# aleju/face-generator

Measured on NVIDIA H100. Metric: 32x32 GAN train images/sec (1 D-iter + 1 G-iter per batch, batch 256/GPU), higher is better.
Workload: dtype f32

## Files before the change

### face_generator_b200/csrc/capi.cu

```cuda
#include <algorithm>
#include <cstdarg>
#include <cstdlib>
#include <cstring>

#include "fg_internal.h"
#include "k_conv_tc.h"

static thread_local char g_err[1024] = "";
void fg_set_error(const char* fmt, ...) {
  va_list ap;
  va_start(ap, fmt);
  vsnprintf(g_err, sizeof(g_err), fmt, ap);
  va_end(ap);
}

#define ENTER(c)                                      \
  do {                                                \
    if (!(c)) {                                       \
      fg_set_error("null fg_ctx");                    \
      return FG_ERR_INVALID;                          \
    }                                                 \
    FG_CUDA(cudaSetDevice((c)->device));              \
  } while (0)

// ... 232 lines not shown
  ENTER(c);
  c->graph_epoch++;
  if (!strcmp(key, "sgd_momentum_D") || !strcmp(key, "sgd_momentum_G")) {
    FG_REQUIRE(v >= 0.0 && v < 1.0, "%s must be in [0, 1)", key);
    (key[13] == 'D' ? c->sgd_mom_D : c->sgd_mom_G) = (float)v;
    return FG_OK;
  }
  fg_set_error("fg_set_option_f: unknown key '%s'", key);
  return FG_ERR_INVALID;
}
int64_t fg_get_option(fg_ctx* c, const char* key) {
  if (!c || !key) return -1;
  if (!strcmp(key, "conv_impl")) return c->conv_impl;
  if (!strcmp(key, "max_batch")) return c->maxB;
  if (!strcmp(key, "channels")) return c->C;
  if (!strcmp(key, "sm_count")) return c->sm_count;
  if (!strcmp(key, "bn_epilogue")) return c->bn_epilogue;
  if (!strcmp(key, "edge_impl")) return c->edge_impl;
  if (!strcmp(key, "mma_f16")) return c->mma_f16;
  if (!strcmp(key, "dp_overlap")) return c->dp_overlap;
  if (!strcmp(key, "use_graph")) return c->use_graph;
  if (!strcmp(key, "bwd_merge")) return c->bwd_merge;
  if (!strcmp(key, "bwd_merge_ctas")) return c->bwd_merge_ctas;
  if (!strcmp(key, "optimizer_D")) return c->opt_D;
  if (!strcmp(key, "optimizer_G")) return c->opt_G;
  if (!strcmp(key, "last_conv_kind")) return c->last_conv_kind;
  if (!strcmp(key, "last_conv_tile_m")) return c->last_conv_tile_m;
  if (!strcmp(key, "last_conv_tile_n")) return c->last_conv_tile_n;
  if (!strcmp(key, "last_conv_format")) return c->last_conv_format;
  if (!strcmp(key, "last_conv_splits")) return c->last_conv_splits;
  return -1;
}

int fg_adam_step(fg_ctx* c, float* p, const float* g, float* m, float* v, int64_t n, float lr, float beta1, float beta2,
                 float eps, int t, float l1_grad, float l2, float clampv, float grad_scale) {
  ENTER(c);
  FG_REQUIRE(p && g && m && v && n > 0 && t >= 1, "fg_adam_step: bad arguments");
  const double step = (double)lr * sqrt(1.0 - pow((double)beta2, t)) / (1.0 - pow((double)beta1, t));
  return k_adam(c, p, g, m, v, n, beta1, beta2, eps, l1_grad, l2, clampv, grad_scale, nullptr, nullptr, (float)step,
                nullptr);
}

void* fg_dev_alloc(size_t bytes) {
  void* p = nullptr;
  if (cudaMalloc(&p, bytes) != cudaSuccess) {
    fg_set_error("fg_dev_alloc(%zu) failed: %s", bytes, cudaGetErrorString(cudaGetLastError()));
// ... 93 lines not shown
```

### face_generator_b200/csrc/fg_internal.h

```cpp
#pragma once
#include <cuda_runtime.h>
#include <cstdint>
#include <cstdio>
#include <deque>
#include <functional>
#include <initializer_list>
#include <map>
#include <string>
#include <vector>

#include "fg_b200.h"

void fg_set_error(const char* fmt, ...);

#define FG_CUDA(call)                                                                               \
  do {                                                                                              \
    cudaError_t e__ = (call);                                                                       \
    if (e__ != cudaSuccess) {                                                                       \
      fg_set_error("%s:%d: %s -> %s", __FILE__, __LINE__, #call, cudaGetErrorString(e__));          \
      return FG_ERR_CUDA;                                                                           \
    }                                                                                               \
  } while (0)
#define FG_TRY(call)                  \
  do {                                \
// ... 192 lines not shown
  double* red_ws = nullptr;
  size_t red_ws_elems = 0;
  double* red_ws_opt = nullptr;
  unsigned* red_ticket = nullptr;
  double* bn_slice_acc = nullptr;
  float* bn_parts = nullptr;
  int edge_impl = 1;
  int bn_epilogue = 1;
  int mma_f16 = 1;
  float* lop_sx = nullptr;
  float* lop_sy = nullptr;
  unsigned* amax_out = nullptr;
  bool* amax_done = nullptr;
  double* bn_acc = nullptr;
  float* io_dev = nullptr;
  size_t io_dev_elems = 0;
  float* scratch[8] = {nullptr, nullptr, nullptr, nullptr, nullptr, nullptr, nullptr, nullptr};
  size_t scratch_elems[8] = {0, 0, 0, 0, 0, 0, 0, 0};
  void* nccl_comm = nullptr;
  int world = 1, rank = 0;
  int dp_overlap = 1;
  int reserve_sms = 0;
  int last_conv_kind = 0, last_conv_tile_m = 0, last_conv_tile_n = 0, last_conv_format = 0, last_conv_splits = 0;
  int bwd_merge = 1, bwd_merge_ctas = 0;
  int* bwd_claim = nullptr;
  int use_graph = 1, graph_epoch = 0;
  uint64_t* seed_dev = nullptr;
  cudaStream_t comm_stream = nullptr;
  cudaEvent_t ev_fork = nullptr, ev_join = nullptr;
  bool debug_keep = false;
  cudaEvent_t events[16] = {};
  bool timing = false;
  std::map<std::string, TimerRec> timers;
};

inline void note_conv(fg_ctx* c, int kind, int tile_m, int tile_n, int format, int splits) {
  c->last_conv_kind = kind;
  c->last_conv_tile_m = tile_m;
  c->last_conv_tile_n = tile_n;
  c->last_conv_format = format;
  c->last_conv_splits = splits;
}

struct ScopedTimer {
  fg_ctx* c;
  TimerRec* rec = nullptr;
  cudaEvent_t e0 = nullptr, e1 = nullptr;
// ... 197 lines not shown
```

### face_generator_b200/csrc/k_conv_tc.cu

```cuda
#include <cuda.h>
#include <cuda_fp16.h>

#include <algorithm>
#include <cstdlib>
#include <cstring>
#include <functional>
#include <queue>
#include <vector>

#include "fg_internal.h"
#include "k_conv_tc.h"
#include "k_f16split.cuh"
#include "k_wgmma.cuh"

namespace {

__device__ __forceinline__ uint32_t smem_u32(const void* p) { return (uint32_t)__cvta_generic_to_shared(p); }

__device__ __forceinline__ void mbar_init(uint64_t* bar, uint32_t count) {
  asm volatile("mbarrier.init.shared::cta.b64 [%0], %1;" ::"r"(smem_u32(bar)), "r"(count));
}
__device__ __forceinline__ void mbar_expect_tx(uint64_t* bar, uint32_t bytes) {
  asm volatile("mbarrier.arrive.expect_tx.shared::cta.b64 _, [%0], %1;" ::"r"(smem_u32(bar)), "r"(bytes) : "memory");
}
// ... 339 lines not shown
bool pick_box(int H, int W, int npix, int* bw, int* bh, int* bb) {
  if (W <= 0 || H <= 0) return false;
  if (W >= npix) {
    if (W % npix) return false;
    *bw = npix; *bh = 1; *bb = 1;
    return true;
  }
  if (npix % W) return false;
  const int rows = npix / W;
  if (rows <= H) {
    if (H % rows) return false;
    *bw = W; *bh = rows; *bb = 1;
    return true;
  }
  if (rows % H) return false;
  *bw = W; *bh = H; *bb = rows / H;
  return true;
}

template <int BN>
constexpr size_t fwd_smem() { return (size_t)kStages * (2 * kABytes + 2 * BN * 128) + 256 + 5 * 8 * BN * 4 + 1024; }
template <int BN>
constexpr size_t wg_smem() { return (size_t)3 * (2 * 4 * 4096 + 2 * (BN / 32) * 4096) + 128 + 1024; }
template <int BN>
constexpr size_t bwd_smem() { return (size_t)kStages * fwd_stage_bytes<BN>() + 256 + 1024; }


template <int N, bool F16 = false>
__global__ void __launch_bounds__(256, 1) tf32_peak_kernel(int iters, float* sink) {
  extern __shared__ uint8_t smem_raw[];
  uint8_t* smem = reinterpret_cast<uint8_t*>((reinterpret_cast<uintptr_t>(smem_raw) + 1023) & ~(uintptr_t)1023);
  constexpr uint32_t kFoot = (128 + N) * 128;
  for (uint32_t i = threadIdx.x; i < kFoot / 4; i += blockDim.x) reinterpret_cast<float*>(smem)[i] = 1.f;
  asm volatile("fence.proxy.async.shared::cta;" ::: "memory");
  __syncthreads();
  const uint32_t sa = smem_u32(smem);
  const uint64_t a = make_desc(sa + (threadIdx.x >> 7) * 64 * 128, 16, 1024), b = make_desc(sa + 128 * 128, 16, 1024);
  float acc[N / 2];
#pragma unroll
  for (int i = 0; i < N / 2; ++i) acc[i] = 0.f;
  for (int i = 0; i < iters; ++i) {
    wgmma_fence();
#pragma unroll
    for (int k = 0; k < 4; ++k) wgmma_op<N, F16, false>(acc, a + (uint64_t)(k * 2), b + (uint64_t)(k * 2), 1);
    wgmma_commit();
    wgmma_wait<1>();
  }
  wgmma_wait<0>();
// ... 31 lines not shown
  cudaEventDestroy(e1);
  const double flops = (double)c->sm_count * iters * 4.0 * 2.0 * 128 * N * (f16 ? 16 : 8);
  *tflops = flops / (best * 1e-3) / 1e12;
  return FG_OK;
}

int tc_encode_nhwc_box(CUtensorMap* m, const float* base, int C, int W, int H, int B, int bc, int bw, int bh, int bb) {
  FG_TRY(get_encode());
  const int64_t sW = (int64_t)C * 4, sH = sW * W, sB = sH * H;
  return make_map4(m, base, C, W, H, B, sW, sH, sB, bc, bw, bh, bb, CU_TENSOR_MAP_SWIZZLE_NONE);
}

int tc_init(fg_ctx* c) {
  (void)c;
  FG_TRY(get_encode());
  FG_CUDA(cudaFuncSetAttribute(tapconv_tc_kernel<64>, cudaFuncAttributeMaxDynamicSharedMemorySize, (int)fwd_smem<64>()));
  FG_CUDA(cudaFuncSetAttribute(tapconv_tc_kernel<128>, cudaFuncAttributeMaxDynamicSharedMemorySize, (int)fwd_smem<128>()));
  FG_CUDA(cudaFuncSetAttribute(tapconv_tc_kernel<64, true>, cudaFuncAttributeMaxDynamicSharedMemorySize, (int)fwd_smem<64>()));
  FG_CUDA(cudaFuncSetAttribute(tapconv_tc_kernel<128, true>, cudaFuncAttributeMaxDynamicSharedMemorySize, (int)fwd_smem<128>()));
  FG_CUDA(cudaFuncSetAttribute(wgrad_tc_kernel<64>, cudaFuncAttributeMaxDynamicSharedMemorySize, (int)wg_smem<64>()));
  FG_CUDA(cudaFuncSetAttribute(wgrad_tc_kernel<128>, cudaFuncAttributeMaxDynamicSharedMemorySize, (int)wg_smem<128>()));
  FG_CUDA(cudaFuncSetAttribute(wgrad_tc_kernel<64, true>, cudaFuncAttributeMaxDynamicSharedMemorySize, (int)wg_smem<64>()));
  FG_CUDA(cudaFuncSetAttribute(wgrad_tc_kernel<128, true>, cudaFuncAttributeMaxDynamicSharedMemorySize, (int)wg_smem<128>()));
  FG_CUDA(cudaFuncSetAttribute(bwd_pair_tc_kernel<128>, cudaFuncAttributeMaxDynamicSharedMemorySize, (int)bwd_smem<128>()));
  return FG_OK;
}
void tc_destroy(fg_ctx* c) { (void)c; }

int tc_split(fg_ctx* c, const float* x, float* hi, float* lo, int64_t n) {
  if (n % 4) {
    fg_set_error("tc_split: element count must be a multiple of 4");
    return FG_ERR_INVALID;
  }
  int64_t g = (n / 4 + 255) / 256;
  if (g > kGridCap) g = kGridCap;
  if (reinterpret_cast<uintptr_t>(x) % 16 == 0) split_kernel<true><<<(int)g, 256, 0, c->stream>>>(x, hi, lo, n / 4);
  else split_kernel<false><<<(int)g, 256, 0, c->stream>>>(x, hi, lo, n / 4);
  LAUNCH_CHECK(c);
  return FG_OK;
}
int tc_amax(fg_ctx* c, const float* x, int64_t n, float* amax_slot) {
  if (n % 4 || reinterpret_cast<uintptr_t>(x) % 16) {
    fg_set_error("tc_amax: needs a 16-byte aligned tensor with a multiple of 4 elements");
    return FG_ERR_INVALID;
  }
  FG_CUDA(cudaMemsetAsync(amax_slot, 0, 2 * sizeof(float), c->stream));
  int64_t g = (n / 4 + 255) / 256;
// ... 179 lines not shown
  FG_TRY(make_map2(&p.b_lo, w_lo, g.Cin, (int64_t)ntapw * g.Cout, ke, BN, false, h));
  p.kpt = g.Cin / ke;
  p.oscale = oscale ? oscale : oscale2;
  p.oscale2 = oscale ? oscale2 : nullptr;
  p.Cout = g.Cout;
  p.B = g.B; p.H = Hl; p.W = Wl;
  p.tiles_x = Wl / p.bw;
  p.tiles_y = Hl / p.bh;
  p.tiles_per_phase = p.bb == 1 ? g.B * p.tiles_x * p.tiles_y : (g.B + p.bb - 1) / p.bb;
  p.out = out;
  p.bias = bias;
  p.stats = stats;
  if (n_parts) *n_parts = p.tiles_per_phase * p.nphase;
  p.out_H = g.H; p.out_W = g.W;
  p.out_scale = g.ups;
  p.ntiles = p.tiles_per_phase * p.nphase * (g.Cout / BN);
  p.chunk = tc_chunk(g.H * g.W > 1);
  if (f16 && g.H * g.W == 1) p.chunk = std::max(1, p.chunk / 2);
  return launch_tapconv(c, p, BN, f16);
}


static int dgrad_ups_params(const float* dy_hi, const float* dy_lo, const float* wd_hi, const float* wd_lo, float* out,
                            ConvGeom g, int f16, const float* oscale, TcFwdParams& p, int* BN_out) {
  memset(&p, 0, sizeof(p));
  const int Hl = g.H / 2, Wl = g.W / 2;
  if (!pick_box(Hl, Wl, 128, &p.bw, &p.bh, &p.bb)) return FG_ERR_UNSUPPORTED;
  const int Cy = g.Cout;
  const int es = f16 ? 2 : 4, ke = f16 ? 64 : 32;
  const bool h = f16 != 0;
  if (Cy % ke) return FG_ERR_UNSUPPORTED;
  for (int ph = 0; ph < 4; ++ph) {
    const int py = ph >> 1, px = ph & 1;
    const int64_t off_bytes = ((int64_t)py * g.W + px) * Cy * es;
    const float* b_hi = reinterpret_cast<const float*>(reinterpret_cast<const char*>(dy_hi) + off_bytes);
    const float* b_lo = reinterpret_cast<const float*>(reinterpret_cast<const char*>(dy_lo) + off_bytes);
    const int64_t sW = (int64_t)2 * Cy * es, sH = (int64_t)2 * g.W * Cy * es, sB = (int64_t)g.H * g.W * Cy * es;
    FG_TRY(make_map4(&p.a_hi[ph], b_hi, Cy, Wl, Hl, g.B, sW, sH, sB, ke, p.bw, p.bh, p.bb, CU_TENSOR_MAP_SWIZZLE_128B, false, h));
    FG_TRY(make_map4(&p.a_lo[ph], b_lo, Cy, Wl, Hl, g.B, sW, sH, sB, ke, p.bw, p.bh, p.bb, CU_TENSOR_MAP_SWIZZLE_128B, false, h));
  }
  const int BN = g.Cin % 128 == 0 ? 128 : 64;
  p.nphase = 1;
  p.ntaps = 36;
  for (int ph = 0; ph < 4; ++ph)
    for (int t = 0; t < 9; ++t) {
      p.dy[ph * 9 + t] = (int8_t)(1 - t / 3);
      p.dx[ph * 9 + t] = (int8_t)(1 - t % 3);
      p.amap[ph * 9 + t] = (int8_t)ph;
      p.widx[ph * 9 + t] = (int16_t)(ph * 9 + t);
    }
  FG_TRY(make_map2(&p.b_hi, wd_hi, Cy, (int64_t)36 * g.Cin, ke, BN, false, h));
  FG_TRY(make_map2(&p.b_lo, wd_lo, Cy, (int64_t)36 * g.Cin, ke, BN, false, h));
  p.kpt = Cy / ke;
  p.oscale = oscale;
  p.Cout = g.Cin;
  p.B = g.B; p.H = Hl; p.W = Wl;
  p.tiles_x = Wl / p.bw;
  p.tiles_y = Hl / p.bh;
  p.tiles_per_phase = p.bb == 1 ? g.B * p.tiles_x * p.tiles_y : (g.B + p.bb - 1) / p.bb;
  p.out = out;
  p.bias = nullptr;
  p.out_H = Hl; p.out_W = Wl;
  p.out_scale = 1;
  p.ntiles = p.tiles_per_phase * (g.Cin / BN);
  p.chunk = tc_chunk(true);
  *BN_out = BN;
  return FG_OK;
}
int tc_conv_dgrad_ups(fg_ctx* c, const float* dy_hi, const float* dy_lo, const float* wd_hi, const float* wd_lo,
                      float* out, ConvGeom g, int f16, const float* oscale) {
  TcFwdParams p;
  int BN;
  FG_TRY(dgrad_ups_params(dy_hi, dy_lo, wd_hi, wd_lo, out, g, f16, oscale, p, &BN));
  return launch_tapconv(c, p, BN, f16);
}

static int wgrad_splits(const fg_ctx* c, int base, int kblocks) {
  const int splits = std::min(std::max(1, c->sm_count / base), kblocks);
  const int per = (kblocks + splits - 1) / splits;
  return (kblocks + per - 1) / per;
}

static int wgrad_params(fg_ctx* c, const float* x_hi, const float* x_lo, const float* dy_hi, const float* dy_lo, ConvGeom g,
                        int f16, const float* oscale, const float* oscale2, TcWgParams& p, int* BN_out, int* ntt_out,
                        int* splits_out) {
  memset(&p, 0, sizeof(p));
  const int Hl = g.H / g.ups, Wl = g.W / g.ups;
  const bool h = f16 != 0;
  const int es = h ? 2 : 4, gch = h ? 64 : 32;
  if (!pick_box(Hl, Wl, h ? 64 : 32, &p.bw, &p.bh, &p.bb)) return FG_ERR_UNSUPPORTED;
  if (g.Cin % 64 || g.Cout % 128) return FG_ERR_UNSUPPORTED;
  const int BN = g.Cin % 128 == 0 ? 128 : 64;
  {
    const int64_t sW = (int64_t)g.Cin * es, sH = sW * Wl, sB = sH * Hl;
    const int ngx = BN / gch;
    FG_TRY(make_map5(&p.x_hi, x_hi, g.Cin, Wl, Hl, g.B, sW, sH, sB, p.bw, p.bh, p.bb, ngx, h));
// ... 63 lines not shown
  if (f16) {
    if (BN == 128) wgrad_tc_kernel<128, true><<<grid, kTcThreads, wg_smem<128>(), c->stream>>>(p);
    else wgrad_tc_kernel<64, true><<<grid, kTcThreads, wg_smem<64>(), c->stream>>>(p);
  } else if (BN == 128) wgrad_tc_kernel<128><<<grid, kTcThreads, wg_smem<128>(), c->stream>>>(p);
  else wgrad_tc_kernel<64><<<grid, kTcThreads, wg_smem<64>(), c->stream>>>(p);
  LAUNCH_CHECK(c);
  return splits > 1 ? k_splitk_reduce(c, c->splitk_ws, splits, size, out) : FG_OK;
}

bool tc_bwd_pair_eligible(const fg_ctx* c, const ConvGeom& g) {
  int bw, bh, bb;
  const int Hl = g.H / 2, Wl = g.W / 2;
  if (g.ups != 2 || g.k != 5 || g.Cin % 128 || g.Cout % 128) return false;
  if (!pick_box(Hl, Wl, 128, &bw, &bh, &bb) || !pick_box(Hl, Wl, 64, &bw, &bh, &bb)) return false;
  const int kblocks = bb == 1 ? g.B * (Wl / bw) * (Hl / bh) : (g.B + bb - 1) / bb;
  return wgrad_splits(c, 36 * (g.Cout / 128) * (g.Cin / 128), kblocks) == 1;
}

static int bwd_pair_ctas(const fg_ctx* c, int nitems) {
  int ctas = std::min(nitems, std::max(1, c->sm_count - c->reserve_sms));
  return c->bwd_merge_ctas > 0 ? std::min(ctas, c->bwd_merge_ctas) : ctas;
}

bool tc_bwd_pair_pays(const fg_ctx* c, const ConvGeom& g) {
  if (!tc_bwd_pair_eligible(c, g)) return false;
  int bw, bh, bb, tw, th, tb;
  const int Hl = g.H / 2, Wl = g.W / 2;
  pick_box(Hl, Wl, 64, &bw, &bh, &bb);
  pick_box(Hl, Wl, 128, &tw, &th, &tb);
  const int64_t wlen = bb == 1 ? g.B * (Wl / bw) * (Hl / bh) : (g.B + bb - 1) / bb;
  const int64_t dlen = 36 * (g.Cout / 64);
  const int nwg = 36 * (g.Cout / 128) * (g.Cin / 128);
  const int ntiles = (tb == 1 ? g.B * (Wl / tw) * (Hl / th) : (g.B + tb - 1) / tb) * (g.Cin / 128);
  const int sms = std::max(1, c->sm_count - c->reserve_sms);
  const int64_t two = wlen + (int64_t)((ntiles + sms - 1) / sms) * dlen;
  std::priority_queue<int64_t, std::vector<int64_t>, std::greater<int64_t>> free_at;
  for (int i = 0, n = bwd_pair_ctas(c, nwg + ntiles); i < n; ++i) free_at.push(0);
  int64_t merged = 0;
  for (int id = 0; id < nwg + ntiles; ++id) {
    const int64_t end = free_at.top() + (id < nwg ? wlen : dlen);
    free_at.pop();
    free_at.push(end);
    merged = std::max(merged, end);
  }
  return merged * 20 < two * 19;
}

int tc_conv_bwd_ups(fg_ctx* c, const float* x_hi, const float* x_lo, const float* dy_hi, const float* dy_lo,
                    const float* wd_hi, const float* wd_lo, float* wg_out, float* dh, ConvGeom g, const float* oscale_dy,
                    const float* oscale_x) {
  if (!tc_bwd_pair_eligible(c, g)) {
    fg_set_error("tc_conv_bwd_ups: no merged backward for Cin %d, Cout %d at %dx%d, batch %d", g.Cin, g.Cout, g.H, g.W, g.B);
    return FG_ERR_UNSUPPORTED;
  }
  TcBwdParams p;
  memset(&p, 0, sizeof(p));
  int wBN, ntt, splits, dBN;
  FG_TRY(wgrad_params(c, x_hi, x_lo, dy_hi, dy_lo, g, 1, oscale_dy, oscale_x, p.wg, &wBN, &ntt, &splits));
  FG_TRY(dgrad_ups_params(dy_hi, dy_lo, wd_hi, wd_lo, dh, g, 1, oscale_dy, p.dg, &dBN));
  if (wBN != 128 || dBN != 128 || splits != 1) {
    fg_set_error("tc_conv_bwd_ups: unexpected tiling (wgrad BN %d, %d splits, dgrad BN %d)", wBN, splits, dBN);
    return FG_ERR_UNSUPPORTED;
  }
  p.wg.out = wg_out;
  p.wg.split_stride = 0;
  p.claim = c->bwd_claim;
  p.nwg = ntt * (g.Cout / 128) * (g.Cin / 128);
  p.nitems = p.nwg + p.dg.ntiles;
  const int ctas = bwd_pair_ctas(c, p.nitems);
  FG_CUDA(cudaMemsetAsync(c->bwd_claim, 0, sizeof(int), c->stream));
  bwd_pair_tc_kernel<128><<<ctas, kTcThreads, bwd_smem<128>(), c->stream>>>(p);
  LAUNCH_CHECK(c);
  return FG_OK;
}
```

### face_generator_b200/csrc/k_conv_tc_kernels.cuh

```cuda
#pragma once

constexpr int kConsumerThreads = 256;
constexpr int kTcThreads = kConsumerThreads + 128;

__device__ __forceinline__ void wgmma_fence() { asm volatile("wgmma.fence.sync.aligned;" ::: "memory"); }
__device__ __forceinline__ void wgmma_commit() { asm volatile("wgmma.commit_group.sync.aligned;" ::: "memory"); }
template <int N>
__device__ __forceinline__ void wgmma_wait() { asm volatile("wgmma.wait_group.sync.aligned %0;" ::"n"(N) : "memory"); }
__device__ __forceinline__ void consumer_sync() { asm volatile("bar.sync 1, %0;" ::"n"(kConsumerThreads) : "memory"); }
__device__ __forceinline__ void producer_regs() { asm volatile("setmaxnreg.dec.sync.aligned.u32 40;" ::: "memory"); }
__device__ __forceinline__ void consumer_regs() { asm volatile("setmaxnreg.inc.sync.aligned.u32 232;" ::: "memory"); }

template <int N, bool F16, bool MN>
__device__ __forceinline__ void wgmma_op(float* d, uint64_t a, uint64_t b, int scale_d) {
  if constexpr (F16) {
    constexpr int T = MN ? 1 : 0;
    if constexpr (N == 64) wgmma_f16_n64<T, T>(d, a, b, scale_d);
    else if constexpr (N == 128) wgmma_f16_n128<T, T>(d, a, b, scale_d);
    else wgmma_f16_n256<T, T>(d, a, b, scale_d);
  } else {
    static_assert(!MN, "tf32 wgmma operands are K-major");
    if constexpr (N == 64) wgmma_tf32_n64(d, a, b, scale_d);
    else if constexpr (N == 128) wgmma_tf32_n128(d, a, b, scale_d);
    else wgmma_tf32_n256(d, a, b, scale_d);
// ... 29 lines not shown
  const int ntn = p.Cout / BN;
  FwdTile t;
  const int mt = tile / ntn;
  t.n0 = (tile - mt * ntn) * BN;
  int r = mt / p.nphase;
  t.ph = mt - r * p.nphase;
  if (p.bb == 1) {
    const int per_img = p.tiles_x * p.tiles_y;
    t.b0 = r / per_img;
    r -= t.b0 * per_img;
    t.y0 = (r / p.tiles_x) * p.bh;
    t.x0 = (r % p.tiles_x) * p.bw;
  } else {
    t.b0 = r * p.bb;
    t.y0 = 0;
    t.x0 = 0;
  }
  return t;
}

template <int BN>
constexpr uint32_t fwd_stage_bytes() { return 2 * kABytes + 2 * BN * 128; }

template <int BN, bool F16>
__device__ __forceinline__ void tapconv_load_tile(const TcFwdParams& p, int tile, uint8_t* smem, uint64_t* full,
                                                  uint64_t* empty, uint32_t& kbg) {
  constexpr uint32_t kBBytes = BN * 128;
  constexpr uint32_t kStageBytes = fwd_stage_bytes<BN>();
  constexpr int kKE = F16 ? 64 : 32;
  const int nkb = p.ntaps * p.kpt;
  const FwdTile t = fwd_decode<BN>(p, tile);
  for (int kb = 0; kb < nkb; ++kb, ++kbg) {
    const uint32_t s = kbg % kStages, it = kbg / kStages;
    if (it > 0) mbar_wait_spin(empty + s, (it - 1) & 1);
    const int tap = kb / p.kpt, c0 = (kb - tap * p.kpt) * kKE;
    const int ti = t.ph * p.ntaps + tap;
    const int am = p.amap[ti];
    uint8_t* st = smem + s * kStageBytes;
    mbar_expect_tx(full + s, kStageBytes);
    tma_load_4d(st, &p.a_hi[am], full + s, c0, t.x0 + p.dx[ti], t.y0 + p.dy[ti], t.b0);
    tma_load_4d(st + kABytes, &p.a_lo[am], full + s, c0, t.x0 + p.dx[ti], t.y0 + p.dy[ti], t.b0);
    const int wrow = p.widx[ti] * p.Cout + t.n0;
    tma_load_2d(st + 2 * kABytes, &p.b_hi, full + s, c0, wrow);
    tma_load_2d(st + 2 * kABytes + kBBytes, &p.b_lo, full + s, c0, wrow);
  }
}

template <int BN, bool F16>
__device__ __forceinline__ void tapconv_mma_tile(const TcFwdParams& p, int tile, uint8_t* smem, uint64_t* full,
                                                 uint64_t* empty, float* stat_sm, uint32_t& kbg) {
  constexpr uint32_t kBBytes = BN * 128;
  constexpr uint32_t kStageBytes = fwd_stage_bytes<BN>();
  const int warp = threadIdx.x >> 5, lane = threadIdx.x & 31;
  const int wg = warp >> 2, g = lane >> 2, tq = lane & 3;
  const uint32_t aoff = (uint32_t)wg * 64 * 128;
  const int nkb = p.ntaps * p.kpt;
  const int kChunk = p.chunk;
  const int nchunks = (nkb + kChunk - 1) / kChunk;
  int rowpix[2];
  for (int h = 0; h < 2; ++h) rowpix[h] = wg * 64 + (warp & 3) * 16 + g + 8 * h;
  float acc[BN];
  const FwdTile t = fwd_decode<BN>(p, tile);
  float o[BN / 2];
#pragma unroll
  for (int i = 0; i < BN / 2; ++i) o[i] = 0.f;
  for (int ch = 0; ch < nchunks; ++ch) {
    const int nk = min(kChunk, nkb - ch * kChunk);
    int prev = -1;
    for (int j = 0; j < nk; ++j, ++kbg) {
      const uint32_t s = kbg % kStages, it = kbg / kStages;
      const uint32_t sa = smem_u32(smem + s * kStageBytes);
      mbar_wait(full + s, it & 1);
      mma_kblock<BN, F16, false>(acc, make_desc(sa + aoff, 16, 1024), make_desc(sa + kABytes + aoff, 16, 1024),
                                 make_desc(sa + 2 * kABytes, 16, 1024), make_desc(sa + 2 * kABytes + kBBytes, 16, 1024),
                                 2, j == 0);
      wgmma_wait<1>();
      if (prev >= 0 && lane == 0) mbar_arrive(empty + prev);
      prev = (int)s;
    }
    wgmma_wait<0>();
    if (lane == 0) mbar_arrive(empty + prev);
    promote<BN, F16>(o, acc);
  }
  if (p.oscale) {
    const float os = *p.oscale * (p.oscale2 ? *p.oscale2 : 1.f);
#pragma unroll
    for (int i = 0; i < BN / 2; ++i) o[i] *= os;
  }
  int b[2];
  float* orow[2];
  for (int h = 0; h < 2; ++h) {
    const int m = rowpix[h];
    const int xi = m % p.bw, yi = (m / p.bw) % p.bh, bi = m / (p.bw * p.bh);
    b[h] = t.b0 + bi;
// ... 84 lines not shown

  if (threadIdx.x == 0) {
    for (int s = 0; s < kStages; ++s) {
      mbar_init(full + s, 1);
      mbar_init(empty + s, kConsumerThreads / 32);
    }
    asm volatile("fence.mbarrier_init.release.cluster;" ::: "memory");
  }
  __syncthreads();

  if (warp >= kConsumerThreads / 32) {
    producer_regs();
    if (warp == kConsumerThreads / 32 && lane == 0) {
      prefetch_tmap(&p.b_hi);
      prefetch_tmap(&p.b_lo);
      uint32_t kbg = 0;
      for (int tile = blockIdx.x; tile < ntiles; tile += gridDim.x) tapconv_load_tile<BN, F16>(p, tile, smem, full, empty, kbg);
    }
    return;
  }

  consumer_regs();
  uint32_t kbg = 0;
  for (int tile = blockIdx.x; tile < ntiles; tile += gridDim.x) tapconv_mma_tile<BN, F16>(p, tile, smem, full, empty, stat_sm, kbg);
}

template <bool F16>
constexpr int wg_stages() { return F16 ? 3 : 2; }

__device__ __forceinline__ uint32_t sw128_off(int n, int k) {
  return (uint32_t)n * 128 + ((uint32_t)((k >> 2) ^ (n & 7)) << 4) + (uint32_t)(k & 3) * 4;
}
__device__ __forceinline__ void transpose_block(const uint8_t* src, uint8_t* dst, int rows, int tid) {
  for (int u = tid; u < rows * 8; u += kConsumerThreads) {
    const int q8 = u & 7, r = u >> 3, px = r & 31, grp = r >> 5;
    const float4 v = *reinterpret_cast<const float4*>(src + ((grp * 32 + px) * 32 + q8 * 4) * 4);
    const int n = grp * 32 + q8 * 4;
    *reinterpret_cast<float*>(dst + sw128_off(n + 0, px)) = v.x;
    *reinterpret_cast<float*>(dst + sw128_off(n + 1, px)) = v.y;
    *reinterpret_cast<float*>(dst + sw128_off(n + 2, px)) = v.z;
    *reinterpret_cast<float*>(dst + sw128_off(n + 3, px)) = v.w;
  }
}

template <int BN, bool F16>
struct WgLayout {
  static constexpr int kS = wg_stages<F16>();
// ... 32 lines not shown
    int b0, y0, x0;
    if (p.bb == 1) {
      const int per_img = p.tiles_x * p.tiles_y;
      b0 = kb / per_img;
      const int r = kb % per_img;
      y0 = (r / p.tiles_x) * p.bh;
      x0 = (r % p.tiles_x) * p.bw;
    } else {
      b0 = kb * p.bb;
      y0 = 0;
      x0 = 0;
    }
    uint8_t* st = smem + s * L::kStageBytes;
    mbar_expect_tx(full + s, L::kStageBytes);
    tma_load_5d(st, &p.dy_hi[ph], full + s, 0, x0, y0, b0, w.m0 / L::kG);
    tma_load_5d(st + L::kAB, &p.dy_lo[ph], full + s, 0, x0, y0, b0, w.m0 / L::kG);
    tma_load_5d(st + 2 * L::kAB, &p.x_hi, full + s, 0, x0 + dxo, y0 + dyo, b0, w.c0 / L::kG);
    tma_load_5d(st + 2 * L::kAB + L::kBB, &p.x_lo, full + s, 0, x0 + dxo, y0 + dyo, b0, w.c0 / L::kG);
  }
}

template <int BN, bool F16>
__device__ __forceinline__ void wgrad_mma_item(const TcWgParams& p, const WgItem& w, uint8_t* smem, uint64_t* full,
                                               uint64_t* empty, uint32_t& kbg) {
  using L = WgLayout<BN, F16>;
  constexpr uint32_t kBox = L::kBox, kAB = L::kAB, kBB = L::kBB;
  uint8_t* kbuf = smem + L::kS * L::kStageBytes;
  const int warp = threadIdx.x >> 5, lane = threadIdx.x & 31;
  const int wg = warp >> 2, g = lane >> 2, tq = lane & 3;
  const int nkb = w.nkb;
  const int kChunk = p.chunk;
  const int nchunks = (nkb + kChunk - 1) / kChunk;
  float acc[BN];
  float o[BN / 2];
#pragma unroll
  for (int i = 0; i < BN / 2; ++i) o[i] = 0.f;
  for (int ch = 0; ch < nchunks; ++ch) {
    const int nk = min(kChunk, nkb - ch * kChunk);
    int prev = -1;
    for (int j = 0; j < nk; ++j, ++kbg) {
      const int s = kbg % L::kS, it = kbg / L::kS;
      const uint32_t sa = smem_u32(smem + s * L::kStageBytes);
      mbar_wait(full + s, it & 1);
      if constexpr (F16) {
        mma_kblock<BN, true, true>(acc, make_desc(sa + wg * kBox, kBox, 1024), make_desc(sa + kAB + wg * kBox, kBox, 1024),
                                   make_desc(sa + 2 * kAB, kBox, 1024), make_desc(sa + 2 * kAB + kBB, kBox, 1024), 128, j == 0);
        wgmma_wait<1>();
        if (prev >= 0 && lane == 0) mbar_arrive(empty + prev);
        prev = s;
      } else {
        const uint8_t* st = smem + s * L::kStageBytes;
        transpose_block(st, kbuf, 128, threadIdx.x);
        transpose_block(st + kAB, kbuf + 128 * 128, 128, threadIdx.x);
        transpose_block(st + 2 * kAB, kbuf + 256 * 128, BN, threadIdx.x);
        transpose_block(st + 2 * kAB + kBB, kbuf + (256 + BN) * 128, BN, threadIdx.x);
        asm volatile("fence.proxy.async.shared::cta;" ::: "memory");
        consumer_sync();
// ... 37 lines not shown
  uint64_t* full = reinterpret_cast<uint64_t*>(smem + (L::kS + (F16 ? 0 : 1)) * L::kStageBytes);
  uint64_t* empty = full + L::kS;

  const int warp = threadIdx.x >> 5, lane = threadIdx.x & 31;
  const WgItem w = wg_decode<BN>(p, blockIdx.x, blockIdx.y, blockIdx.z);

  if (threadIdx.x == 0) {
    for (int s = 0; s < L::kS; ++s) {
      mbar_init(full + s, 1);
      mbar_init(empty + s, kConsumerThreads / 32);
    }
    asm volatile("fence.mbarrier_init.release.cluster;" ::: "memory");
  }
  __syncthreads();
  if (w.nkb <= 0) return;

  uint32_t kbg = 0;
  if (warp >= kConsumerThreads / 32) {
    producer_regs();
    if (warp == kConsumerThreads / 32 && lane == 0) wgrad_load_item<BN, F16>(p, w, smem, full, empty, kbg);
    return;
  }
  consumer_regs();
  wgrad_mma_item<BN, F16>(p, w, smem, full, empty, kbg);
}

constexpr int kIdSlots = 2;

template <int BN>
__global__ void __launch_bounds__(kTcThreads, 1) bwd_pair_tc_kernel(const __grid_constant__ TcBwdParams p) {
  using L = WgLayout<BN, true>;
  static_assert(L::kS == kStages && L::kStageBytes == fwd_stage_bytes<BN>(), "one stage ring for both item kinds");
  extern __shared__ uint8_t smem_raw[];
  uint8_t* smem = reinterpret_cast<uint8_t*>((reinterpret_cast<uintptr_t>(smem_raw) + 1023) & ~(uintptr_t)1023);
  uint64_t* full = reinterpret_cast<uint64_t*>(smem + kStages * L::kStageBytes);
  uint64_t* empty = full + kStages;
  uint64_t* id_full = empty + kStages;
  uint64_t* id_empty = id_full + kIdSlots;
  volatile int* ids = reinterpret_cast<volatile int*>(id_empty + kIdSlots);

  const int warp = threadIdx.x >> 5, lane = threadIdx.x & 31;
  const int nmn = (p.wg.Cout / 128) * (p.wg.Cin / BN);

  if (threadIdx.x == 0) {
    for (int s = 0; s < kStages; ++s) {
      mbar_init(full + s, 1);
      mbar_init(empty + s, kConsumerThreads / 32);
    }
    for (int s = 0; s < kIdSlots; ++s) {
      mbar_init(id_full + s, 1);
      mbar_init(id_empty + s, kConsumerThreads / 32);
    }
    asm volatile("fence.mbarrier_init.release.cluster;" ::: "memory");
  }
  __syncthreads();

  uint32_t kbg = 0;
  if (warp >= kConsumerThreads / 32) {
    producer_regs();
    if (warp == kConsumerThreads / 32 && lane == 0) {
      prefetch_tmap(&p.dg.b_hi);
      prefetch_tmap(&p.dg.b_lo);
      for (uint32_t n = 0;; ++n) {
        const uint32_t slot = n % kIdSlots, use = n / kIdSlots;
        if (use > 0) mbar_wait_spin(id_empty + slot, (use - 1) & 1);
        const int id = atomicAdd(p.claim, 1);
        ids[slot] = id;
        mbar_arrive(id_full + slot);
        if (id >= p.nitems) break;
        if (id < p.nwg) wgrad_load_item<BN, true>(p.wg, wg_decode<BN>(p.wg, id / nmn, id % nmn, 0), smem, full, empty, kbg);
        else tapconv_load_tile<BN, true>(p.dg, id - p.nwg, smem, full, empty, kbg);
      }
    }
    return;
  }

  consumer_regs();
  for (uint32_t n = 0;; ++n) {
    const uint32_t slot = n % kIdSlots, use = n / kIdSlots;
    mbar_wait(id_full + slot, use & 1);
    const int id = ids[slot];
    __syncwarp();
    if (lane == 0) mbar_arrive(id_empty + slot);
    if (id >= p.nitems) break;
    if (id < p.nwg) wgrad_mma_item<BN, true>(p.wg, wg_decode<BN>(p.wg, id / nmn, id % nmn, 0), smem, full, empty, kbg);
    else tapconv_mma_tile<BN, true>(p.dg, id - p.nwg, smem, full, empty, nullptr, kbg);
  }
}
```

### face_generator_b200/csrc/nets_s16.cu

```cuda
#include <algorithm>

#include "fg_internal.h"
#include "k_misc.h"
#include "ups_gan.h"

namespace {
constexpr int kS16Mask = 1024 + 128;
constexpr int kSide = 16;

__global__ void avgpool2_fwd_kernel(const float* __restrict__ x, float* __restrict__ y, int B, int H, int W, int C) {
  const int Ho = H / 2, Wo = W / 2;
  const int64_t n = (int64_t)B * Ho * Wo * C;
  GRID_STRIDE(i, n) {
    const int ch = (int)(i % C);
    int64_t r = i / C;
    const int xo = (int)(r % Wo); r /= Wo;
    const int yo = (int)(r % Ho);
    const int64_t b = r / Ho;
    const float* p = x + (((b * H + 2 * yo) * W + 2 * xo) * (int64_t)C + ch);
    y[i] = 0.25f * ((p[0] + p[C]) + (p[(int64_t)W * C] + p[(int64_t)W * C + C]));
  }
}
__global__ void avgpool2_bwd_kernel(const float* __restrict__ dy, float* __restrict__ dx, int B, int H, int W, int C) {
  const int Ho = H / 2, Wo = W / 2;
// ... 286 lines not shown
}

struct fg_s16 : UpsGan {};

#define ENTER(n)                                         \
  do {                                                   \
    if (!(n) || !(n)->c) {                               \
      fg_set_error("null fg_s16");                       \
      return FG_ERR_INVALID;                             \
    }                                                    \
    FG_CUDA(cudaSetDevice((n)->c->device));              \
  } while (0)

extern "C" {

int fg_s16_create(fg_ctx* ctx, fg_s16** out) {
  if (!ctx || !out) {
    fg_set_error("fg_s16_create: null argument");
    return FG_ERR_INVALID;
  }
  *out = nullptr;
  FG_CUDA(cudaSetDevice(ctx->device));
  fg_s16* n = new fg_s16();
  static const GanDesc k16{{kSide, "s16.", 0, false}, kS16Mask, false};
  const int r = gan_alloc(*n, ctx, k16, std::make_unique<D16>(), nullptr);
  if (r != FG_OK) {
    fg_s16_destroy(n);
    return r;
  }
  *out = n;
  return FG_OK;
}
int fg_s16_destroy(fg_s16* n) {
  if (!n) return FG_OK;
  if (n->c) {
    cudaSetDevice(n->c->device);
    cudaStreamSynchronize(n->c->stream);
  }
  gan_free(*n);
  delete n;
  return FG_OK;
}
int64_t fg_s16_param_count(int net, int channels) {
  if (net != FG_NET_D) return make_g_layout(channels, kSide).total;
  return D16().layout(channels);
}
int fg_s16_mask_per_sample(void) { return kS16Mask; }
// ... 103 lines not shown
```

Measured before the change: 37440.

## Let merged backward kernel pick dgrad tile width 64 via schedule cost model

The fused wgrad+dgrad backward kernel is templated on the dgrad tile width. A list-scheduling cost model compares BN=128 against BN=64, using a fixed per-tile cost ratio, and launches the variant with the smaller predicted makespan. BN=64 gives more, smaller dgrad tiles to balance load across CTAs in the persistent queue. Accumulator arrays are hoisted out of the item functions so both item kinds share registers, and a flag in the s16 net descriptor is also flipped. A profiling script measures the BN=64 cost ratio.

```diff
diff --git a/face_generator_b200/csrc/capi.cu b/face_generator_b200/csrc/capi.cu
--- a/face_generator_b200/csrc/capi.cu
+++ b/face_generator_b200/csrc/capi.cu
@@ -278,6 +278,7 @@
   if (!strcmp(key, "use_graph")) return c->use_graph;
   if (!strcmp(key, "bwd_merge")) return c->bwd_merge;
   if (!strcmp(key, "bwd_merge_ctas")) return c->bwd_merge_ctas;
+  if (!strcmp(key, "last_bwd_merge_tile_n")) return c->bwd_merge_tile_n;
   if (!strcmp(key, "optimizer_D")) return c->opt_D;
   if (!strcmp(key, "optimizer_G")) return c->opt_G;
   if (!strcmp(key, "last_conv_kind")) return c->last_conv_kind;
diff --git a/face_generator_b200/csrc/fg_internal.h b/face_generator_b200/csrc/fg_internal.h
--- a/face_generator_b200/csrc/fg_internal.h
+++ b/face_generator_b200/csrc/fg_internal.h
@@ -238,7 +238,7 @@
   int dp_overlap = 1;
   int reserve_sms = 0;
   int last_conv_kind = 0, last_conv_tile_m = 0, last_conv_tile_n = 0, last_conv_format = 0, last_conv_splits = 0;
-  int bwd_merge = 1, bwd_merge_ctas = 0;
+  int bwd_merge = 1, bwd_merge_ctas = 0, bwd_merge_tile_n = 0;
   int* bwd_claim = nullptr;
   int use_graph = 1, graph_epoch = 0;
   uint64_t* seed_dev = nullptr;
diff --git a/face_generator_b200/csrc/k_conv_tc.cu b/face_generator_b200/csrc/k_conv_tc.cu
--- a/face_generator_b200/csrc/k_conv_tc.cu
+++ b/face_generator_b200/csrc/k_conv_tc.cu
@@ -385,8 +385,7 @@
 constexpr size_t fwd_smem() { return (size_t)kStages * (2 * kABytes + 2 * BN * 128) + 256 + 5 * 8 * BN * 4 + 1024; }
 template <int BN>
 constexpr size_t wg_smem() { return (size_t)3 * (2 * 4 * 4096 + 2 * (BN / 32) * 4096) + 128 + 1024; }
-template <int BN>
-constexpr size_t bwd_smem() { return (size_t)kStages * fwd_stage_bytes<BN>() + 256 + 1024; }
+constexpr size_t bwd_smem() { return (size_t)kStages * fwd_stage_bytes<128>() + 256 + 1024; }
 
 
 template <int N, bool F16 = false>
@@ -464,7 +463,8 @@
   FG_CUDA(cudaFuncSetAttribute(wgrad_tc_kernel<128>, cudaFuncAttributeMaxDynamicSharedMemorySize, (int)wg_smem<128>()));
   FG_CUDA(cudaFuncSetAttribute(wgrad_tc_kernel<64, true>, cudaFuncAttributeMaxDynamicSharedMemorySize, (int)wg_smem<64>()));
   FG_CUDA(cudaFuncSetAttribute(wgrad_tc_kernel<128, true>, cudaFuncAttributeMaxDynamicSharedMemorySize, (int)wg_smem<128>()));
-  FG_CUDA(cudaFuncSetAttribute(bwd_pair_tc_kernel<128>, cudaFuncAttributeMaxDynamicSharedMemorySize, (int)bwd_smem<128>()));
+  FG_CUDA(cudaFuncSetAttribute(bwd_pair_tc_kernel<64>, cudaFuncAttributeMaxDynamicSharedMemorySize, (int)bwd_smem()));
+  FG_CUDA(cudaFuncSetAttribute(bwd_pair_tc_kernel<128>, cudaFuncAttributeMaxDynamicSharedMemorySize, (int)bwd_smem()));
   return FG_OK;
 }
 void tc_destroy(fg_ctx* c) { (void)c; }
@@ -690,8 +690,9 @@
 
 
 static int dgrad_ups_params(const float* dy_hi, const float* dy_lo, const float* wd_hi, const float* wd_lo, float* out,
-                            ConvGeom g, int f16, const float* oscale, TcFwdParams& p, int* BN_out) {
+                            ConvGeom g, int f16, const float* oscale, int BN, TcFwdParams& p) {
   memset(&p, 0, sizeof(p));
+  if (g.Cin % BN) return FG_ERR_UNSUPPORTED;
   const int Hl = g.H / 2, Wl = g.W / 2;
   if (!pick_box(Hl, Wl, 128, &p.bw, &p.bh, &p.bb)) return FG_ERR_UNSUPPORTED;
   const int Cy = g.Cout;
@@ -707,7 +708,6 @@
     FG_TRY(make_map4(&p.a_hi[ph], b_hi, Cy, Wl, Hl, g.B, sW, sH, sB, ke, p.bw, p.bh, p.bb, CU_TENSOR_MAP_SWIZZLE_128B, false, h));
     FG_TRY(make_map4(&p.a_lo[ph], b_lo, Cy, Wl, Hl, g.B, sW, sH, sB, ke, p.bw, p.bh, p.bb, CU_TENSOR_MAP_SWIZZLE_128B, false, h));
   }
-  const int BN = g.Cin % 128 == 0 ? 128 : 64;
   p.nphase = 1;
   p.ntaps = 36;
   for (int ph = 0; ph < 4; ++ph)
@@ -732,14 +732,14 @@
   p.out_scale = 1;
   p.ntiles = p.tiles_per_phase * (g.Cin / BN);
   p.chunk = tc_chunk(true);
-  *BN_out = BN;
   return FG_OK;
 }
 int tc_conv_dgrad_ups(fg_ctx* c, const float* dy_hi, const float* dy_lo, const float* wd_hi, const float* wd_lo,
                       float* out, ConvGeom g, int f16, const float* oscale) {
+  static const int force64 = getenv("FG_TC_DGRAD_BN") && atoi(getenv("FG_TC_DGRAD_BN")) == 64;
+  const int BN = g.Cin % 128 == 0 && !force64 ? 128 : 64;
   TcFwdParams p;
-  int BN;
-  FG_TRY(dgrad_ups_params(dy_hi, dy_lo, wd_hi, wd_lo, out, g, f16, oscale, p, &BN));
+  FG_TRY(dgrad_ups_params(dy_hi, dy_lo, wd_hi, wd_lo, out, g, f16, oscale, BN, p));
   return launch_tapconv(c, p, BN, f16);
 }
 
@@ -849,28 +849,43 @@
   return c->bwd_merge_ctas > 0 ? std::min(ctas, c->bwd_merge_ctas) : ctas;
 }
 
-bool tc_bwd_pair_pays(const fg_ctx* c, const ConvGeom& g) {
-  if (!tc_bwd_pair_eligible(c, g)) return false;
+constexpr double kDgradBn64Cost = 0.67;
+
+static double pair_schedule(int ctas, int nwg, double wlen, int ndg, double dlen) {
+  std::priority_queue<double, std::vector<double>, std::greater<double>> free_at;
+  for (int i = 0; i < ctas; ++i) free_at.push(0.0);
+  double end = 0.0;
+  for (int id = 0; id < nwg + ndg; ++id) {
+    const double t = free_at.top() + (id < nwg ? wlen : dlen);
+    free_at.pop();
+    free_at.push(t);
+    end = std::max(end, t);
+  }
+  return end;
+}
+
+static int bwd_pair_plan(const fg_ctx* c, const ConvGeom& g, bool* pays) {
   int bw, bh, bb, tw, th, tb;
   const int Hl = g.H / 2, Wl = g.W / 2;
   pick_box(Hl, Wl, 64, &bw, &bh, &bb);
   pick_box(Hl, Wl, 128, &tw, &th, &tb);
-  const int64_t wlen = bb == 1 ? g.B * (Wl / bw) * (Hl / bh) : (g.B + bb - 1) / bb;
-  const int64_t dlen = 36 * (g.Cout / 64);
+  const double wlen = bb == 1 ? g.B * (Wl / bw) * (Hl / bh) : (g.B + bb - 1) / bb;
+  const double dlen = 36 * (g.Cout / 64);
   const int nwg = 36 * (g.Cout / 128) * (g.Cin / 128);
-  const int ntiles = (tb == 1 ? g.B * (Wl / tw) * (Hl / th) : (g.B + tb - 1) / tb) * (g.Cin / 128);
+  const int mt = tb == 1 ? g.B * (Wl / tw) * (Hl / th) : (g.B + tb - 1) / tb;
+  const int n128 = mt * (g.Cin / 128), n64 = mt * (g.Cin / 64);
   const int sms = std::max(1, c->sm_count - c->reserve_sms);
-  const int64_t two = wlen + (int64_t)((ntiles + sms - 1) / sms) * dlen;
-  std::priority_queue<int64_t, std::vector<int64_t>, std::greater<int64_t>> free_at;
-  for (int i = 0, n = bwd_pair_ctas(c, nwg + ntiles); i < n; ++i) free_at.push(0);
-  int64_t merged = 0;
-  for (int id = 0; id < nwg + ntiles; ++id) {
-    const int64_t end = free_at.top() + (id < nwg ? wlen : dlen);
-    free_at.pop();
-    free_at.push(end);
-    merged = std::max(merged, end);
-  }
-  return merged * 20 < two * 19;
+  const double two = wlen + (double)((n128 + sms - 1) / sms) * dlen;
+  const double m128 = pair_schedule(bwd_pair_ctas(c, nwg + n128), nwg, wlen, n128, dlen);
+  const double m64 = pair_schedule(bwd_pair_ctas(c, nwg + n64), nwg, wlen, n64, kDgradBn64Cost * dlen);
+  *pays = m128 * 20 < two * 19;
+  return m64 < m128 ? 64 : 128;
+}
+
+bool tc_bwd_pair_pays(const fg_ctx* c, const ConvGeom& g) {
+  bool pays = false;
+  if (tc_bwd_pair_eligible(c, g)) bwd_pair_plan(c, g, &pays);
+  return pays;
 }
 
 int tc_conv_bwd_ups(fg_ctx* c, const float* x_hi, const float* x_lo, const float* dy_hi, const float* dy_lo,
@@ -882,11 +897,13 @@
   }
   TcBwdParams p;
   memset(&p, 0, sizeof(p));
-  int wBN, ntt, splits, dBN;
+  bool pays;
+  const int dBN = bwd_pair_plan(c, g, &pays);
+  int wBN, ntt, splits;
   FG_TRY(wgrad_params(c, x_hi, x_lo, dy_hi, dy_lo, g, 1, oscale_dy, oscale_x, p.wg, &wBN, &ntt, &splits));
-  FG_TRY(dgrad_ups_params(dy_hi, dy_lo, wd_hi, wd_lo, dh, g, 1, oscale_dy, p.dg, &dBN));
-  if (wBN != 128 || dBN != 128 || splits != 1) {
-    fg_set_error("tc_conv_bwd_ups: unexpected tiling (wgrad BN %d, %d splits, dgrad BN %d)", wBN, splits, dBN);
+  FG_TRY(dgrad_ups_params(dy_hi, dy_lo, wd_hi, wd_lo, dh, g, 1, oscale_dy, dBN, p.dg));
+  if (wBN != 128 || splits != 1) {
+    fg_set_error("tc_conv_bwd_ups: unexpected tiling (wgrad BN %d, %d splits)", wBN, splits);
     return FG_ERR_UNSUPPORTED;
   }
   p.wg.out = wg_out;
@@ -896,7 +913,9 @@
   p.nitems = p.nwg + p.dg.ntiles;
   const int ctas = bwd_pair_ctas(c, p.nitems);
   FG_CUDA(cudaMemsetAsync(c->bwd_claim, 0, sizeof(int), c->stream));
-  bwd_pair_tc_kernel<128><<<ctas, kTcThreads, bwd_smem<128>(), c->stream>>>(p);
-  LAUNCH_CHECK(c);
-  return FG_OK;
-}
+  c->bwd_merge_tile_n = dBN;
+  if (dBN == 64) bwd_pair_tc_kernel<64><<<ctas, kTcThreads, bwd_smem(), c->stream>>>(p);
+  else bwd_pair_tc_kernel<128><<<ctas, kTcThreads, bwd_smem(), c->stream>>>(p);
+  LAUNCH_CHECK(c);
+  return FG_OK;
+}
diff --git a/face_generator_b200/csrc/k_conv_tc_kernels.cuh b/face_generator_b200/csrc/k_conv_tc_kernels.cuh
--- a/face_generator_b200/csrc/k_conv_tc_kernels.cuh
+++ b/face_generator_b200/csrc/k_conv_tc_kernels.cuh
@@ -75,7 +75,7 @@
 template <int BN>
 constexpr uint32_t fwd_stage_bytes() { return 2 * kABytes + 2 * BN * 128; }
 
-template <int BN, bool F16>
+template <int BN, bool F16, uint32_t kStride = fwd_stage_bytes<BN>()>
 __device__ __forceinline__ void tapconv_load_tile(const TcFwdParams& p, int tile, uint8_t* smem, uint64_t* full,
                                                   uint64_t* empty, uint32_t& kbg) {
   constexpr uint32_t kBBytes = BN * 128;
@@ -89,7 +89,7 @@
     const int tap = kb / p.kpt, c0 = (kb - tap * p.kpt) * kKE;
     const int ti = t.ph * p.ntaps + tap;
     const int am = p.amap[ti];
-    uint8_t* st = smem + s * kStageBytes;
+    uint8_t* st = smem + s * kStride;
     mbar_expect_tx(full + s, kStageBytes);
     tma_load_4d(st, &p.a_hi[am], full + s, c0, t.x0 + p.dx[ti], t.y0 + p.dy[ti], t.b0);
     tma_load_4d(st + kABytes, &p.a_lo[am], full + s, c0, t.x0 + p.dx[ti], t.y0 + p.dy[ti], t.b0);
@@ -99,11 +99,11 @@
   }
 }
 
-template <int BN, bool F16>
+template <int BN, bool F16, uint32_t kStride = fwd_stage_bytes<BN>()>
 __device__ __forceinline__ void tapconv_mma_tile(const TcFwdParams& p, int tile, uint8_t* smem, uint64_t* full,
-                                                 uint64_t* empty, float* stat_sm, uint32_t& kbg) {
+                                                 uint64_t* empty, float* stat_sm, uint32_t& kbg, float (&acc)[BN],
+                                                 float (&o)[BN / 2]) {
   constexpr uint32_t kBBytes = BN * 128;
-  constexpr uint32_t kStageBytes = fwd_stage_bytes<BN>();
   const int warp = threadIdx.x >> 5, lane = threadIdx.x & 31;
   const int wg = warp >> 2, g = lane >> 2, tq = lane & 3;
   const uint32_t aoff = (uint32_t)wg * 64 * 128;
@@ -112,9 +112,7 @@
   const int nchunks = (nkb + kChunk - 1) / kChunk;
   int rowpix[2];
   for (int h = 0; h < 2; ++h) rowpix[h] = wg * 64 + (warp & 3) * 16 + g + 8 * h;
-  float acc[BN];
   const FwdTile t = fwd_decode<BN>(p, tile);
-  float o[BN / 2];
 #pragma unroll
   for (int i = 0; i < BN / 2; ++i) o[i] = 0.f;
   for (int ch = 0; ch < nchunks; ++ch) {
@@ -122,7 +120,7 @@
     int prev = -1;
     for (int j = 0; j < nk; ++j, ++kbg) {
       const uint32_t s = kbg % kStages, it = kbg / kStages;
-      const uint32_t sa = smem_u32(smem + s * kStageBytes);
+      const uint32_t sa = smem_u32(smem + s * kStride);
       mbar_wait(full + s, it & 1);
       mma_kblock<BN, F16, false>(acc, make_desc(sa + aoff, 16, 1024), make_desc(sa + kABytes + aoff, 16, 1024),
                                  make_desc(sa + 2 * kABytes, 16, 1024), make_desc(sa + 2 * kABytes + kBBytes, 16, 1024),
@@ -253,7 +251,10 @@
 
   consumer_regs();
   uint32_t kbg = 0;
-  for (int tile = blockIdx.x; tile < ntiles; tile += gridDim.x) tapconv_mma_tile<BN, F16>(p, tile, smem, full, empty, stat_sm, kbg);
+  for (int tile = blockIdx.x; tile < ntiles; tile += gridDim.x) {
+    float acc[BN], o[BN / 2];
+    tapconv_mma_tile<BN, F16>(p, tile, smem, full, empty, stat_sm, kbg, acc, o);
+  }
 }
 
 template <bool F16>
@@ -332,7 +333,7 @@
 
 template <int BN, bool F16>
 __device__ __forceinline__ void wgrad_mma_item(const TcWgParams& p, const WgItem& w, uint8_t* smem, uint64_t* full,
-                                               uint64_t* empty, uint32_t& kbg) {
+                                               uint64_t* empty, uint32_t& kbg, float (&acc)[BN], float (&o)[BN / 2]) {
   using L = WgLayout<BN, F16>;
   constexpr uint32_t kBox = L::kBox, kAB = L::kAB, kBB = L::kBB;
   uint8_t* kbuf = smem + L::kS * L::kStageBytes;
@@ -341,8 +342,6 @@
   const int nkb = w.nkb;
   const int kChunk = p.chunk;
   const int nchunks = (nkb + kChunk - 1) / kChunk;
-  float acc[BN];
-  float o[BN / 2];
 #pragma unroll
   for (int i = 0; i < BN / 2; ++i) o[i] = 0.f;
   for (int ch = 0; ch < nchunks; ++ch) {
@@ -426,15 +425,18 @@
     return;
   }
   consumer_regs();
-  wgrad_mma_item<BN, F16>(p, w, smem, full, empty, kbg);
+  float acc[BN], o[BN / 2];
+  wgrad_mma_item<BN, F16>(p, w, smem, full, empty, kbg, acc, o);
 }
 
 constexpr int kIdSlots = 2;
 
-template <int BN>
+template <int DBN>
 __global__ void __launch_bounds__(kTcThreads, 1) bwd_pair_tc_kernel(const __grid_constant__ TcBwdParams p) {
+  constexpr int BN = 128;
   using L = WgLayout<BN, true>;
-  static_assert(L::kS == kStages && L::kStageBytes == fwd_stage_bytes<BN>(), "one stage ring for both item kinds");
+  static_assert(L::kS == kStages && L::kStageBytes == fwd_stage_bytes<BN>() && fwd_stage_bytes<DBN>() <= L::kStageBytes,
+                "one stage ring for both item kinds");
   extern __shared__ uint8_t smem_raw[];
   uint8_t* smem = reinterpret_cast<uint8_t*>((reinterpret_cast<uintptr_t>(smem_raw) + 1023) & ~(uintptr_t)1023);
   uint64_t* full = reinterpret_cast<uint64_t*>(smem + kStages * L::kStageBytes);
@@ -473,13 +475,14 @@
         mbar_arrive(id_full + slot);
         if (id >= p.nitems) break;
         if (id < p.nwg) wgrad_load_item<BN, true>(p.wg, wg_decode<BN>(p.wg, id / nmn, id % nmn, 0), smem, full, empty, kbg);
-        else tapconv_load_tile<BN, true>(p.dg, id - p.nwg, smem, full, empty, kbg);
+        else tapconv_load_tile<DBN, true, L::kStageBytes>(p.dg, id - p.nwg, smem, full, empty, kbg);
       }
     }
     return;
   }
 
   consumer_regs();
+  float acc[BN], o[BN / 2];
   for (uint32_t n = 0;; ++n) {
     const uint32_t slot = n % kIdSlots, use = n / kIdSlots;
     mbar_wait(id_full + slot, use & 1);
@@ -487,7 +490,9 @@
     __syncwarp();
     if (lane == 0) mbar_arrive(id_empty + slot);
     if (id >= p.nitems) break;
-    if (id < p.nwg) wgrad_mma_item<BN, true>(p.wg, wg_decode<BN>(p.wg, id / nmn, id % nmn, 0), smem, full, empty, kbg);
-    else tapconv_mma_tile<BN, true>(p.dg, id - p.nwg, smem, full, empty, nullptr, kbg);
-  }
-}
+    if (id < p.nwg) wgrad_mma_item<BN, true>(p.wg, wg_decode<BN>(p.wg, id / nmn, id % nmn, 0), smem, full, empty, kbg, acc, o);
+    else tapconv_mma_tile<DBN, true, L::kStageBytes>(p.dg, id - p.nwg, smem, full, empty, nullptr, kbg,
+                                                     reinterpret_cast<float(&)[DBN]>(acc),
+                                                     reinterpret_cast<float(&)[DBN / 2]>(o));
+  }
+}
diff --git a/face_generator_b200/csrc/nets_s16.cu b/face_generator_b200/csrc/nets_s16.cu
--- a/face_generator_b200/csrc/nets_s16.cu
+++ b/face_generator_b200/csrc/nets_s16.cu
@@ -332,7 +332,7 @@
   *out = nullptr;
   FG_CUDA(cudaSetDevice(ctx->device));
   fg_s16* n = new fg_s16();
-  static const GanDesc k16{{kSide, "s16.", 0, false}, kS16Mask, false};
+  static const GanDesc k16{{kSide, "s16.", 0, true}, kS16Mask, false};
   const int r = gan_alloc(*n, ctx, k16, std::make_unique<D16>(), nullptr);
   if (r != FG_OK) {
     fg_s16_destroy(n);
diff --git a/profiles/dgrad_bn.py b/profiles/dgrad_bn.py
--- /dev/null
+++ b/profiles/dgrad_bn.py
@@ -0,0 +1,76 @@
+import argparse
+import json
+import os
+import subprocess
+import sys
+
+import numpy as np
+
+ROOT = os.path.dirname(os.path.dirname(os.path.abspath(__file__)))
+sys.path.insert(0, ROOT)
+
+
+def gpu_info():
+    try:
+        out = subprocess.run(["nvidia-smi", "--query-gpu=name,power.limit", "--format=csv,noheader"],
+                             capture_output=True, text=True, timeout=30).stdout.strip().splitlines()
+        return out[0] if out else "unknown"
+    except (OSError, subprocess.SubprocessError):
+        return "unknown"
+
+
+def child(B, steps):
+    import face_generator_b200 as fg
+    from face_generator_b200 import layouts as LY
+    from face_generator_b200.lib import NET_D, NET_G
+    C = 3
+    rng = np.random.default_rng(1)
+    ctx = fg.Context(0, max_batch=B, channels=C)
+    ctx.set_option("bwd_merge", 0)
+    ctx.set_params(NET_G, LY.trained_like_init(LY.G_layout(C), rng))
+    ctx.set_params(NET_D, LY.trained_like_init(LY.D_layout(C), rng, 1.4))
+    f = lambda a: np.ascontiguousarray(a, np.float32)
+    real = ctx.dev_array(f(rng.random((B // 2, C, 32, 32))))
+    nD, nG = ctx.dev_array(f(rng.uniform(-1, 1, (B // 2, 100)))), ctx.dev_array(f(rng.uniform(-1, 1, (B, 100))))
+    h = fg.hyper_default()
+    for i in range(5):
+        ctx.train_step(h, B, real, nD, nG, None, None, i + 1, want_stats=False)
+    ctx.timing_enable(True)
+    for i in range(steps):
+        ctx.train_step(h, B, real, nD, nG, None, None, i + 10, want_stats=False)
+    ctx.sync()
+    t, n = ctx.timing_get("G.C1.dgrad")
+    ctx.timing_enable(False)
+    print(json.dumps({"ms": t / steps, "launches": n, "sms": ctx.get_option("sm_count")}))
+    ctx.close()
+
+
+def main():
+    ap = argparse.ArgumentParser()
+    ap.add_argument("--batch", type=int, default=256)
+    ap.add_argument("--steps", type=int, default=20)
+    ap.add_argument("--rounds", type=int, default=3)
+    ap.add_argument("--child", action="store_true")
+    a = ap.parse_args()
+    if a.child:
+        return child(a.batch, a.steps)
+    ms = {128: [], 64: []}
+    sms = 0
+    for _ in range(a.rounds):
+        for bn in (128, 64):
+            env = dict(os.environ, FG_TC_DGRAD_BN=str(bn))
+            out = subprocess.run([sys.executable, os.path.abspath(__file__), "--child", "--batch", str(a.batch),
+                                  "--steps", str(a.steps)], env=env, capture_output=True, text=True, check=True).stdout
+            r = json.loads(out.strip().splitlines()[-1])
+            ms[bn].append(r["ms"])
+            sms = r["sms"]
+    tiles = {bn: (a.batch * 64 + 127) // 128 * (128 // bn) for bn in (128, 64)}
+    waves = {bn: (tiles[bn] + sms - 1) // sms for bn in (128, 64)}
+    per_wave = {bn: float(np.median(ms[bn])) / waves[bn] for bn in (128, 64)}
+    print(json.dumps({"gpu": gpu_info(), "batch": a.batch, "steps": a.steps, "sms": sms, "tiles": tiles, "waves": waves,
+                      "G.C1.dgrad_ms": {bn: [round(x, 4) for x in v] for bn, v in ms.items()},
+                      "bn64_kblock_cost": round(per_wave[64] / per_wave[128], 3)}, indent=1))
+
+
+if __name__ == "__main__":
+    main()
```

New measurement: 37340 (median of 6 runs). No clear change (-0.3%).
